# JohannesBuchner/massivedatans

Measured on AMD Instinct MI355X. Metric: likelihood evals/sec across N datasets per constrained draw, higher is better.
Workload: dtype f64

## Files before the change

include/mdns.h:

```cpp
#ifndef MDNS_H
#define MDNS_H

#include <stddef.h>
#include <stdint.h>

#ifdef __cplusplus
extern "C" {
#endif


int mdns_init(int device);
int mdns_device_count(void);
const char *mdns_last_error(void);
int mdns_abi_version(void);


int mdns_gauss_like(const void *x, const void *yy, int ndata, int nx,
                    double A, double mu, double sig, double noise_level,
                    const void *data_mask, void *Lout);

int mdns_muse_like(const void *yy, const void *vv, const void *ypred, const void *data_mask,
                   int ndata, int nx, void *Lout);

int mdns_register_spectra(const void *yy, const void *vv, int ndata, int nx);
// ... 33 lines not shown
int mdns_lines_loglike_batch(mdns_spectra *s, const double *params, int B,
                             const int *row_ids, int M, double *Lout);
int mdns_lines_template_batch(mdns_spectra *s, const double *params, int B, double *out);

int mdns_curve_loglike_batch(mdns_spectra *s, const double *curves, int B, double noise_level,
                             const int *row_ids, int M, double *Lout);

typedef struct mdns_region mdns_region;

mdns_region *mdns_region_create(const double *members, int K, int ndim);
mdns_region *mdns_region_create_bootstrapped(const double *members, int K, int ndim,
                                             const unsigned *packed, int nbootstraps, double *radius);
mdns_region *mdns_region_wrap_dev(const double *d_members, int K, int ndim);
void mdns_region_destroy(mdns_region *r);
double mdns_region_bootstrap_radius(mdns_region *r, const double *chosen, int nbootstraps);
double mdns_region_bootstrap_radius_dev(mdns_region *r, const double *d_chosen, int nbootstraps);
double mdns_region_bootstrap_radius_packed(mdns_region *r, const unsigned *packed, int nbootstraps);
int mdns_region_bootstrap_radius_async(mdns_region *r, const double *d_chosen, int nbootstraps);
int mdns_region_set_radius(mdns_region *r, double maxdistance);
double mdns_region_radius(mdns_region *r);
int mdns_region_count(mdns_region *r, const double *points, int M, int *counts);
int mdns_region_count_dev(mdns_region *r, const double *d_points, int M, int *d_counts);
int mdns_region_count_polled(mdns_region *r, const double *points, int M, int *counts);


typedef struct mdns_joint mdns_joint;

mdns_joint *mdns_joint_create(mdns_spectra *s, int nlive, int shelf_cap);
void mdns_joint_destroy(mdns_joint *j);

int mdns_joint_init_gauss(mdns_joint *j, const double *params, double noise_level);
int mdns_joint_init_muse3(mdns_joint *j, const double *params, const double *jitter);
int mdns_joint_init_curves(mdns_joint *j, const double *curves, double noise_level, const double *jitter);
int mdns_joint_set_live(mdns_joint *j, const double *liveL);
int mdns_joint_get_live(mdns_joint *j, double *liveL);

int mdns_joint_set_running(mdns_joint *j, const int *rows, int nrun);

int mdns_joint_prepare(mdns_joint *j, double *Lmin, int *argmin, unsigned long long *keep);
int mdns_joint_keep_words(const mdns_joint *j);
int mdns_joint_advance(mdns_joint *j);
int mdns_joint_reserve(mdns_joint *j, int shelf_cap);
int mdns_joint_shelf_cap(const mdns_joint *j);

int mdns_joint_draw_gauss(mdns_joint *j, const double *params, int B, double noise_level,
                          const int *row_ids, int M, int *accepted, double *Lrow,
                          unsigned long long *fillbits);
#define MDNS_JOINT_MAX_BATCH 1024
int mdns_joint_score(mdns_joint *j, const double *params, int B, double noise_level,
                     const int *row_ids, int M);
int mdns_joint_commit(mdns_joint *j, int *accepted, double *Lrow, unsigned long long *fillbits);

int mdns_joint_get_thresholds(mdns_joint *j, double *higher, int *shelf_n);


void *mdns_dev_alloc(size_t bytes);
void mdns_dev_free(void *p);
int mdns_h2d(void *dst, const void *src, size_t bytes);
int mdns_d2h(void *dst, const void *src, size_t bytes);
int mdns_d2d(void *dst, const void *src, size_t bytes);
int mdns_sync(void);
int mdns_set_stream(void *hip_stream);

void *mdns_event_create(void);
void mdns_event_destroy(void *ev);
int mdns_event_record(void *ev);
double mdns_event_elapsed_ms(void *ev_start, void *ev_stop);

int mdns_profile(int classes);
int mdns_profile_every(int n);
int mdns_profile_read(int which, long long *launches, double *total_ms);
const char *mdns_profile_kernel(int which);

int mdns_gauss_loglike_batch_dev(mdns_spectra *s, const double *d_params, int B,
                                 double noise_level, const int *d_row_ids, int M,
                                 double *d_Lout);
int mdns_muse_loglike_batch_dev(mdns_spectra *s, const double *d_ypred, int B,
                                const int *d_row_ids, int M, double *d_Lout);
int mdns_muse3_loglike_batch_dev(mdns_spectra *s, const double *d_params, int B,
                                 const int *d_row_ids, int M, double *d_Lout);
int mdns_lines_loglike_batch_dev(mdns_spectra *s, const double *d_params, int B,
                                 const int *d_row_ids, int M, double *d_Lout);

int mdns_curve_loglike_batch_dev(mdns_spectra *s, const double *d_curves, int ldc, int B, double noise_level,
                                 const int *d_row_ids, int M, double *d_Lout);

int mdns_joint_score_dev(mdns_joint *j, const double *d_params, int B, double noise_level,
                         const int *d_row_ids, int M);
int *mdns_joint_flags_dev(mdns_joint *j);
int mdns_joint_commit_dev(mdns_joint *j, const int *d_row_ids, int M);
int mdns_joint_commit_bits_dev(mdns_joint *j, const int *d_row_ids, int M);
const void *mdns_joint_result_dev(mdns_joint *j);
size_t mdns_joint_result_bytes(int M);
int mdns_joint_fetch(mdns_joint *j, int M, int *accepted, unsigned long long *fillbits);
int mdns_joint_prepare_dev(mdns_joint *j);
int mdns_joint_advance_dev(mdns_joint *j);
int mdns_joint_restore_live_dev(mdns_joint *j, const double *d_liveL);
int mdns_joint_undo_advance_dev(mdns_joint *j);
const double *mdns_joint_live_dev(mdns_joint *j);

int mdns_count_within_dev(const double *d_members, int K, int ndim, double maxdistance,
                          const double *d_cands, int M, int *d_counts);
int mdns_bootstrap_round_maxsq_dev(const double *d_members, int K, int ndim,
                                   const double *d_chosen, int nbootstraps,
                                   double *d_round_sq);

// ... 254 lines not shown
```

massivedatans_amd/_lib.py:

```python
import ctypes as C
import os

import numpy as np

PKG_DIR = os.path.dirname(os.path.abspath(__file__))
LIB_PATH = os.path.join(PKG_DIR, "libmdns_hip.so")
DROPIN_DIR = os.path.join(PKG_DIR, "dropin")

ABI_SYMBOLS = (
    "mdns_init", "mdns_device_count", "mdns_last_error", "mdns_abi_version",
    "mdns_gauss_like", "mdns_muse_like", "mdns_register_spectra", "mdns_unregister_spectra",
    "mdns_most_distant_nearest_neighbor", "mdns_is_within_distance_of",
    "mdns_count_within_distance_of", "mdns_bootstrapped_maxdistance",
    "mdns_spectra_create", "mdns_spectra_destroy", "mdns_spectra_ndata", "mdns_spectra_nx",
    "mdns_gauss_loglike_batch", "mdns_muse_loglike_batch", "mdns_muse3_loglike_batch",
    "mdns_region_create", "mdns_region_create_bootstrapped", "mdns_region_wrap_dev", "mdns_region_destroy",
    "mdns_region_bootstrap_radius", "mdns_region_bootstrap_radius_dev", "mdns_region_bootstrap_radius_packed",
    "mdns_region_bootstrap_radius_async", "mdns_region_set_radius",
    "mdns_region_radius", "mdns_region_count", "mdns_region_count_dev", "mdns_region_count_polled",
    "mdns_dev_alloc", "mdns_dev_free", "mdns_h2d", "mdns_d2h", "mdns_d2d", "mdns_sync", "mdns_set_stream",
    "mdns_event_create", "mdns_event_destroy", "mdns_event_record", "mdns_event_elapsed_ms",
    "mdns_profile", "mdns_profile_every", "mdns_profile_read", "mdns_profile_kernel",
    "mdns_gauss_loglike_batch_dev", "mdns_muse_loglike_batch_dev", "mdns_muse3_loglike_batch_dev",
    "mdns_count_within_dev", "mdns_bootstrap_round_maxsq_dev",
    "mdns_joint_create", "mdns_joint_destroy", "mdns_joint_init_gauss", "mdns_joint_init_muse3", "mdns_joint_set_live",
    "mdns_joint_get_live", "mdns_joint_set_running", "mdns_joint_prepare", "mdns_joint_keep_words",
    "mdns_joint_advance", "mdns_joint_reserve", "mdns_joint_shelf_cap", "mdns_joint_draw_gauss", "mdns_joint_score", "mdns_joint_commit",
    "mdns_joint_get_thresholds", "mdns_joint_score_dev", "mdns_joint_flags_dev", "mdns_joint_commit_dev", "mdns_joint_commit_bits_dev",
    "mdns_joint_result_dev", "mdns_joint_result_bytes", "mdns_joint_fetch", "mdns_joint_prepare_dev", "mdns_joint_advance_dev",
    "mdns_joint_restore_live_dev", "mdns_joint_undo_advance_dev", "mdns_joint_live_dev",
    "mdns_groups_create", "mdns_groups_destroy", "mdns_groups_set_ids", "mdns_groups_get_ids",
    "mdns_groups_replace", "mdns_groups_components", "mdns_groups_labels", "mdns_groups_id_labels", "mdns_groups_mean_rounds",
    "mdns_backend_region_create", "mdns_backend_region_destroy", "mdns_backend_region_count",
    "mdns_backend_draw_begin", "mdns_backend_draw_chunk", "mdns_backend_chunk_size",
    "mdns_backend_region_begin", "mdns_backend_region_radius", "mdns_backend_chain_begin", "mdns_backend_chain_end",
    "mdns_backend_draw_score", "mdns_joint_votes_dev", "mdns_backend_draw_commit", "mdns_get_stream",
    "mdns_backend_draw_band", "mdns_backend_draw_band_commit", "mdns_muse_filter_mode", "mdns_muse_filter_stats", "mdns_muse_filter_dev",
    "mdns_backend_draw_band_begin", "mdns_backend_draw_band_ready", "mdns_backend_draw_band_end",
    "mdns_posterior_create", "mdns_posterior_destroy", "mdns_posterior_summary", "mdns_posterior_resample",
    "mdns_posterior_timings",
    "mdns_spectra_set_lines", "mdns_spectra_nparams", "mdns_lines_loglike_batch", "mdns_lines_loglike_batch_dev",
    "mdns_lines_template_batch",
    "mdns_curve_loglike_batch", "mdns_curve_loglike_batch_dev", "mdns_joint_init_curves",
    "mdns_backend_draw_curves", "mdns_backend_draw_curves_dev",
    "mdns_spectra_set_continuum", "mdns_spectra_continuum", "mdns_muse_continuum_fit_batch", "mdns_muse_continuum_fit_batch_dev",
    "mdns_curve_chi2_batch", "mdns_curve_chi2_batch_dev", "mdns_spectra_set_fixed_scale", "mdns_spectra_fixed_scale",
    "mdns_spectra_set_counts", "mdns_spectra_counts", "mdns_curve_poisson_batch", "mdns_curve_poisson_batch_dev",
    "mdns_spectra_set_background", "mdns_spectra_background", "mdns_curve_wstat_batch", "mdns_curve_wstat_batch_dev",
    "mdns_curve_background_batch", "mdns_curve_background_batch_dev",
    "mdns_table_create", "mdns_table_create_los", "mdns_table_destroy", "mdns_table_nparams", "mdns_table_nx", "mdns_table_curves_batch",
    "mdns_table_curves_batch_dev", "mdns_backend_draw_table", "mdns_joint_init_table",
    "mdns_response_create", "mdns_response_destroy", "mdns_response_nx", "mdns_response_nin", "mdns_response_fold_batch",
    "mdns_response_fold_batch_dev", "mdns_spectra_set_response",
    "mdns_sum_create", "mdns_sum_add_table", "mdns_sum_add_powerlaw", "mdns_sum_add_gauss", "mdns_sum_set_attenuation",
    "mdns_sum_destroy", "mdns_sum_nparams", "mdns_sum_nx", "mdns_sum_ncomponents", "mdns_sum_curves_batch",
    "mdns_sum_curves_batch_dev", "mdns_backend_draw_sum", "mdns_joint_init_sum",
)

HOST_ABI_SYMBOLS = (
    "mdns_constrainer_create", "mdns_constrainer_destroy", "mdns_constrainer_forget_region",
    "mdns_constrainer_draw", "mdns_constrainer_stats", "mdns_constrainer_share_stats", "mdns_host_last_error",
    "mdns_host_rng_get_gauss", "mdns_host_rng_set_gauss",
    "mdns_core_create", "mdns_core_destroy", "mdns_core_last_error", "mdns_core_set_host_edges", "mdns_core_set_incremental",
    "mdns_core_set_initial",
    "mdns_core_purge", "mdns_core_fill", "mdns_core_advance", "mdns_core_cut_down", "mdns_core_npoints",
    "mdns_core_nrunning", "mdns_core_pile_u", "mdns_core_pile_x", "mdns_core_get_ids", "mdns_core_get_shelves",
    "mdns_core_get_superpoints", "mdns_core_stats",
)

JOINT_MAX_BATCH = 1024
TABLE_MAX_AXES = 4
TABLE_TILE = 256
TABLE_REDSHIFT = 1
TABLE_AMPLITUDE = 2
TABLE_EXTINCTION = 4
TABLE_BROADEN = 8
TABLE_BROADEN_CUT = 5.0
TABLE_BROADEN_C = float.fromhex("-0x1.bcb7b1526e50ep-3")
SUM_MAX_COMPONENTS = 8


# ... 27 lines not shown
        "mdns_spectra_nx": (i, [vp]),
        "mdns_gauss_loglike_batch": (i, [vp, vp, i, d, vp, i, vp]),
        "mdns_muse_loglike_batch": (i, [vp, vp, i, vp, i, vp]),
        "mdns_muse3_loglike_batch": (i, [vp, vp, i, vp, i, vp]),
        "mdns_region_create": (vp, [vp, i, i]),
        "mdns_region_create_bootstrapped": (vp, [vp, i, i, vp, i, vp]),
        "mdns_region_wrap_dev": (vp, [vp, i, i]),
        "mdns_region_destroy": (None, [vp]),
        "mdns_region_bootstrap_radius": (d, [vp, vp, i]),
        "mdns_region_bootstrap_radius_dev": (d, [vp, vp, i]),
        "mdns_region_bootstrap_radius_packed": (d, [vp, vp, i]),
        "mdns_region_bootstrap_radius_async": (i, [vp, vp, i]),
        "mdns_region_set_radius": (i, [vp, d]),
        "mdns_region_radius": (d, [vp]),
        "mdns_region_count": (i, [vp, vp, i, vp]),
        "mdns_region_count_dev": (i, [vp, vp, i, vp]),
        "mdns_region_count_polled": (i, [vp, vp, i, vp]),
        "mdns_dev_alloc": (vp, [sz]),
        "mdns_dev_free": (None, [vp]),
        "mdns_h2d": (i, [vp, vp, sz]),
        "mdns_d2h": (i, [vp, vp, sz]),
        "mdns_d2d": (i, [vp, vp, sz]),
        "mdns_sync": (i, []),
        "mdns_set_stream": (i, [vp]),
        "mdns_event_create": (vp, []),
        "mdns_event_destroy": (None, [vp]),
        "mdns_event_record": (i, [vp]),
        "mdns_event_elapsed_ms": (d, [vp, vp]),
        "mdns_profile": (i, [i]),
        "mdns_profile_every": (i, [i]),
        "mdns_profile_read": (i, [i, vp, vp]),
        "mdns_profile_kernel": (C.c_char_p, [i]),
        "mdns_gauss_loglike_batch_dev": (i, [vp, vp, i, d, vp, i, vp]),
        "mdns_muse_loglike_batch_dev": (i, [vp, vp, i, vp, i, vp]),
        "mdns_muse3_loglike_batch_dev": (i, [vp, vp, i, vp, i, vp]),
        "mdns_count_within_dev": (i, [vp, i, i, d, vp, i, vp]),
        "mdns_bootstrap_round_maxsq_dev": (i, [vp, i, i, vp, i, vp]),
        "mdns_joint_create": (vp, [vp, i, i]),
        "mdns_joint_destroy": (None, [vp]),
        "mdns_joint_init_gauss": (i, [vp, vp, d]),
        "mdns_joint_init_muse3": (i, [vp, vp, vp]),
        "mdns_joint_set_live": (i, [vp, vp]),
        "mdns_joint_get_live": (i, [vp, vp]),
        "mdns_joint_set_running": (i, [vp, vp, i]),
        "mdns_joint_prepare": (i, [vp, vp, vp, vp]),
        "mdns_joint_keep_words": (i, [vp]),
        "mdns_joint_advance": (i, [vp]),
        "mdns_joint_reserve": (i, [vp, i]),
        "mdns_joint_shelf_cap": (i, [vp]),
        "mdns_joint_draw_gauss": (i, [vp, vp, i, d, vp, i, vp, vp, vp]),
        "mdns_joint_score": (i, [vp, vp, i, d, vp, i]),
        "mdns_joint_commit": (i, [vp, vp, vp, vp]),
        "mdns_joint_get_thresholds": (i, [vp, vp, vp]),
        "mdns_joint_score_dev": (i, [vp, vp, i, d, vp, i]),
        "mdns_joint_flags_dev": (vp, [vp]),
        "mdns_joint_commit_dev": (i, [vp, vp, i]),
        "mdns_joint_commit_bits_dev": (i, [vp, vp, i]),
        "mdns_joint_result_dev": (vp, [vp]),
        "mdns_joint_result_bytes": (sz, [i]),
        "mdns_joint_fetch": (i, [vp, i, vp, vp]),
        "mdns_joint_prepare_dev": (i, [vp]),
        "mdns_joint_advance_dev": (i, [vp]),
        "mdns_joint_restore_live_dev": (i, [vp, vp]),
        "mdns_joint_undo_advance_dev": (i, [vp]),
        "mdns_joint_live_dev": (vp, [vp]),
        "mdns_groups_create": (vp, [i, i]),
        "mdns_groups_destroy": (None, [vp]),
        "mdns_groups_set_ids": (i, [vp, vp]),
        "mdns_groups_get_ids": (i, [vp, vp]),
        "mdns_groups_replace": (i, [vp, vp, vp, vp, i]),
        "mdns_groups_components": (i, [vp, vp, i, C.c_longlong, vp, vp, vp, C.c_longlong, vp]),
        "mdns_groups_labels": (i, [vp, vp, vp]),
        "mdns_groups_id_labels": (i, [vp, vp, vp, C.c_longlong]),
        "mdns_groups_mean_rounds": (d, [vp]),
        "mdns_backend_region_create": (vp, [vp, vp, i, i, vp, i, vp]),
        "mdns_backend_region_destroy": (None, [vp, vp]),
        "mdns_backend_region_count": (i, [vp, vp, vp, i, vp]),
        "mdns_backend_draw_begin": (i, [vp, vp, i]),
        "mdns_backend_draw_chunk": (i, [vp, vp, i, vp, vp, vp, vp]),
        "mdns_backend_chunk_size": (i, [vp, i, i, i]),
        "mdns_backend_region_begin": (vp, [vp, vp, i, i, vp, i]),
        "mdns_backend_region_radius": (i, [vp, vp, vp]),
        "mdns_backend_draw_score": (i, [vp, vp, i, vp]),
        "mdns_joint_votes_dev": (vp, [vp]),
        "mdns_backend_draw_commit": (i, [vp, vp, vp]),
        "mdns_get_stream": (vp, []),
        "mdns_backend_draw_band": (i, [vp, vp, i, vp, vp, vp, vp, vp, vp, vp, i]),
        "mdns_backend_draw_band_commit": (i, [vp, i, vp, vp]),
        "mdns_backend_draw_band_begin": (i, [vp, vp, i, vp]),
        "mdns_backend_draw_band_ready": (i, [vp]),
        "mdns_backend_draw_band_end": (i, [vp, vp, vp, vp, vp, vp, vp, i]),
        "mdns_muse_filter_dev": (i, [vp, vp, i, vp, i, vp, vp, vp]),
        "mdns_muse_filter_mode": (None, [i]),
        "mdns_muse_filter_stats": (None, [vp]),
        "mdns_posterior_create": (vp, [vp, vp, vp, i, i, i]),
        "mdns_posterior_destroy": (None, [vp]),
        "mdns_posterior_summary": (i, [vp, vp, i, vp, vp, vp, vp, vp, vp, vp]),
        "mdns_posterior_resample": (i, [vp, C.c_ulonglong, C.c_longlong, i, vp, vp]),
        "mdns_posterior_timings": (i, [vp, vp]),
        "mdns_spectra_set_lines": (i, [vp, vp, i, i]),
        "mdns_spectra_nparams": (i, [vp]),
        "mdns_lines_loglike_batch": (i, [vp, vp, i, vp, i, vp]),
        "mdns_lines_loglike_batch_dev": (i, [vp, vp, i, vp, i, vp]),
        "mdns_lines_template_batch": (i, [vp, vp, i, vp]),
        "mdns_curve_loglike_batch": (i, [vp, vp, i, d, vp, i, vp]),
        "mdns_curve_loglike_batch_dev": (i, [vp, vp, i, i, d, vp, i, vp]),
# ... 99 lines not shown
```

massivedatans_amd/csrc/mdns_core.hip:

```cpp
#include "mdns_internal.h"
#include <time.h>

#include <atomic>
#include <cmath>
#include <cstdarg>
#include <cstdio>
#include <cstdlib>
#include <cstring>
#include <mutex>
#include <vector>

namespace mdns {

static char g_error[512] = "";

void set_error(const char *fmt, ...)
{
	va_list ap;
	va_start(ap, fmt);
	vsnprintf(g_error, sizeof(g_error), fmt, ap);
	va_end(ap);
	if (getenv("MDNS_VERBOSE")) fprintf(stderr, "[mdns] %s\n", g_error);
}

// ... 215 lines not shown
	return MDNS_HIP(hipStreamSynchronize(c->stream)) ? 0 : 1;
}
extern "C" int mdns_set_stream(void *hip_stream)
{
	Context *c = ctx();
	if (!c) return 1;
	c->stream = hip_stream ? (hipStream_t) hip_stream : c->own_stream;
	return 0;
}
extern "C" void *mdns_get_stream(void)
{
	Context *c = ctx();
	return c ? (void *) c->stream : nullptr;
}
extern "C" void *mdns_event_create(void)
{
	if (!ctx()) return nullptr;
	hipEvent_t ev;
	if (!MDNS_HIP(hipEventCreate(&ev))) return nullptr;
	return (void *) ev;
}
extern "C" void mdns_event_destroy(void *ev) { if (ev) (void) hipEventDestroy((hipEvent_t) ev); }
extern "C" int mdns_event_record(void *ev)
{
	Context *c = ctx();
	if (!c || !ev) return 1;
	return MDNS_HIP(hipEventRecord((hipEvent_t) ev, c->stream)) ? 0 : 1;
}
extern "C" double mdns_event_elapsed_ms(void *a, void *b)
{
	if (!a || !b) return NAN;
	if (!MDNS_HIP(hipEventSynchronize((hipEvent_t) b))) return NAN;
	float ms = 0;
	if (!MDNS_HIP(hipEventElapsedTime(&ms, (hipEvent_t) a, (hipEvent_t) b))) return NAN;
	return (double) ms;
}

extern "C" int mdns_profile(int classes)
{
	if (!ctx()) return 1;
	drain_pending();
	for (int k = 0; k < 4; k++)
		if (classes & (1 << k)) { g_prof_count[k] = 0; g_prof_ms[k] = 0; g_prof_seen[k] = 0; }
	g_profiling = classes & 15;
	return 0;
}
extern "C" int mdns_profile_every(int n)
{
	g_prof_every = n > 1 ? n : 1;
	return 0;
}
static constexpr int kNoteArgs = 4;
struct KernelNote { const char *fmt; int narg; int num[kNoteArgs]; const char *str[kNoteArgs]; };
static KernelNote g_kernel_note[4];
static char g_kernel_name[4][64];
void mdns::note_kernel(int which, const char *fmt, ...)
{
	if (which < 0 || which > 3) return;
	KernelNote &n = g_kernel_note[which];
	n.fmt = fmt;
	n.narg = 0;
	va_list ap;
	va_start(ap, fmt);
	for (const char *p = fmt; *p && n.narg < kNoteArgs; p++) {
		if (*p != '%') continue;
		if (!*++p) break;
		if (*p == 'd') { n.str[n.narg] = nullptr; n.num[n.narg++] = va_arg(ap, int); }
		else if (*p == 's') { n.num[n.narg] = 0; n.str[n.narg++] = va_arg(ap, const char *); }
	}
	va_end(ap);
}
extern "C" const char *mdns_profile_kernel(int which)
{
	if (which < 0 || which > 3) return "";
	const KernelNote &n = g_kernel_note[which];
	char *out = g_kernel_name[which];
	const size_t cap = sizeof g_kernel_name[which];
	size_t len = 0;
	int a = 0;
	out[0] = 0;
	for (const char *p = n.fmt; p && *p && len + 1 < cap; p++) {
		if (*p == '%' && (p[1] == 'd' || p[1] == 's') && a < n.narg) {
			const int w = n.str[a] ? snprintf(out + len, cap - len, "%s", n.str[a]) : snprintf(out + len, cap - len, "%d", n.num[a]);
			len = w < 0 || len + (size_t) w >= cap ? cap - 1 : len + (size_t) w;
			a++;
			p++;
		} else {
			out[len++] = *p;
			out[len] = 0;
		}
	}
	return out;
}
extern "C" int mdns_profile_read(int which, long long *launches, double *total_ms)
{
	if (!ctx() || which < 0 || which > 3) return 1;
	drain_pending();
	if (launches) *launches = g_prof_count[which];
	if (total_ms) *total_ms = g_prof_ms[which];
	return 0;
}

static bool upload_rows(const double *h_src, int ndata, int nx, int layout, double *d_dst, int ld,
                        bool invert)
{
	Context *c = ctx();
	const size_t n = (size_t) ndata * nx;
	DeviceBuffer<double> tmp;
	if (!tmp.make(n)) return false;
	double *const d_tmp = tmp.get();
	bool ok = MDNS_HIP(hipMemcpyAsync(d_tmp, h_src, n * sizeof(double), hipMemcpyHostToDevice, c->stream));
	if (ok) {
		if (layout == MDNS_LAYOUT_CHANNEL_MAJOR) ok = launch_transpose(d_tmp, nx, ndata, d_dst, ld, invert, ndata);
		else ok = launch_copy_rows(d_tmp, nx, ndata, d_dst, ld, invert);
	}
	return MDNS_HIP(hipStreamSynchronize(c->stream)) && ok;
}

extern "C" mdns_spectra *mdns_spectra_create(const double *x, const double *y, const double *v,
                                             int ndata, int nx, int layout)
{
	Context *c = ctx();
	if (!c) return nullptr;
	if (ndata < 0 || nx < 0 || !y || (layout != 0 && layout != 1)) {
		set_error("mdns_spectra_create: bad arguments (ndata=%d nx=%d layout=%d)", ndata, nx, layout);
		return nullptr;
	}
// ... 855 lines not shown
```

massivedatans_amd/csrc/mdns_joint.hip:

```cpp
#include "mdns_internal.h"

#include <cmath>
#include <cstring>
#include <vector>

namespace mdns {

static constexpr int kBlock = 256;
static constexpr int kFlagInts = MDNS_JOINT_MAX_BATCH;
static constexpr int kZeroInts = kFlagInts + (int) (sizeof(JointHeader) / sizeof(int));

static constexpr int kSlices = 16, kHeld = 8;

template <typename T, typename F> __device__ __forceinline__ T over_slices(T v, F f)
{
	v = f(v, __shfl_xor(v, 4));
	v = f(v, __shfl_xor(v, 8));
	v = f(v, __shfl_xor(v, 16));
	v = f(v, __shfl_xor(v, 32));
	return v;
}

__global__ __launch_bounds__(kBlock) void k_joint_prepare(JointArrays st, const int *__restrict__ running, int nrun,
                                                          double *__restrict__ Lmin, int *__restrict__ argmin_run,
// ... 603 lines not shown
	if (j->stat == kCurveNoise) j->noise_level = noise_level;
	if (!sum_curves(j, c, m, params, j->nlive)) return 1;
	return init_from_curves(j, c, jitter);
}

extern "C" int mdns_joint_restore_live_dev(mdns_joint *j, const double *d_liveL)
{
	Context *c = ctx();
	if (!c || !j || !d_liveL) return 1;
	if (!MDNS_HIP(hipMemcpyAsync(j->st.live, d_liveL, (size_t) j->nlive * j->ndata * sizeof(double), hipMemcpyDeviceToDevice, c->stream))) return 1;
	return joint_reset(j);
}

extern "C" int mdns_joint_undo_advance_dev(mdns_joint *j)
{
	Context *c = ctx();
	if (!c || !j) return 1;
	if (!j->prepared) { set_error("mdns_joint_undo_advance_dev: nothing to take back"); return 1; }
	if (j->nrun == 0) return 0;
	joint_new_epoch(j);
	hipLaunchKernelGGL(k_joint_undo_advance, dim3((j->nrun + kBlock - 1) / kBlock), dim3(kBlock), 0, c->stream,
	                   j->st, j->d_running.get(), j->nrun, j->d_argmin.get(), j->d_Lmin.get());
	return MDNS_HIP(hipGetLastError()) ? 0 : 1;
}

extern "C" const double *mdns_joint_live_dev(mdns_joint *j) { return j ? j->st.live : nullptr; }

extern "C" int mdns_joint_set_live(mdns_joint *j, const double *liveL)
{
	Context *c = ctx();
	if (!c || !j || !liveL) return 1;
	if (!MDNS_HIP(hipMemcpyAsync(j->st.live, liveL, (size_t) j->nlive * j->ndata * sizeof(double), hipMemcpyHostToDevice, c->stream))) return 1;
	if (joint_reset(j) != 0) return 1;
	return joint_sync(c) ? 0 : 1;
}

extern "C" int mdns_joint_get_live(mdns_joint *j, double *liveL)
{
	Context *c = ctx();
	if (!c || !j || !liveL) return 1;
	if (!MDNS_HIP(hipMemcpyAsync(liveL, j->st.live, (size_t) j->nlive * j->ndata * sizeof(double), hipMemcpyDeviceToHost, c->stream))) return 1;
	return joint_sync(c) ? 0 : 1;
}

extern "C" int mdns_joint_get_thresholds(mdns_joint *j, double *higher, int *shelf_n)
{
	Context *c = ctx();
	if (!c || !j) return 1;
	if (higher && !MDNS_HIP(hipMemcpyAsync(higher, j->st.higher, (size_t) j->ndata * sizeof(double), hipMemcpyDeviceToHost, c->stream))) return 1;
	if (shelf_n && !MDNS_HIP(hipMemcpyAsync(shelf_n, j->st.shelfn, (size_t) j->ndata * sizeof(int), hipMemcpyDeviceToHost, c->stream))) return 1;
	return joint_sync(c) ? 0 : 1;
}

extern "C" int mdns_joint_set_running(mdns_joint *j, const int *rows, int nrun)
{
	Context *c = ctx();
	if (!c || !j) return 1;
	if (nrun < 0 || nrun > j->ndata || (nrun > 0 && !rows)) { set_error("mdns_joint_set_running: nrun=%d", nrun); return 1; }
	for (int i = 0; i < nrun; i++)
		if (rows[i] < 0 || rows[i] >= j->ndata || (i > 0 && rows[i] <= rows[i - 1])) {
			set_error("mdns_joint_set_running: rows must be ascending indices below %d", j->ndata);
			return 1;
		}
	if (nrun > 0 && (!MDNS_HIP(hipMemcpyAsync(j->d_running.get(), rows, (size_t) nrun * sizeof(int), hipMemcpyHostToDevice, c->stream)) ||
	                 !joint_sync(c))) return 1;
	j->nrun = nrun;
	return 0;
}

extern "C" int mdns_joint_prepare_dev(mdns_joint *j)
{
	Context *c = ctx();
	if (!c || !j) return 1;
	const int kw = keep_words_of(j->cap);
	if (!j->d_keep.fit((size_t) j->ndata * kw)) return 1;
	j->prepared = true;
	if (j->nrun == 0) return 0;
	joint_new_epoch(j);
	hipLaunchKernelGGL(k_joint_prepare, dim3((j->nrun + 15) / 16), dim3(kBlock), 0, c->stream,
	                   j->st, j->d_running.get(), j->nrun, j->d_Lmin.get(), j->d_argmin_run.get(), j->d_argmin.get(), j->d_keep.get(), kw);
	return MDNS_HIP(hipGetLastError()) ? 0 : 1;
}

extern "C" int mdns_joint_prepare(mdns_joint *j, double *Lmin, int *argmin, unsigned long long *keep)
{
	Context *c = ctx();
	if (mdns_joint_prepare_dev(j) != 0) return 1;
	const int kw = keep_words_of(j->cap);
	const size_t n = (size_t) j->nrun;
	if (n == 0) return 0;
	const size_t o1 = n * 8, o2 = o1 + ((n * 4 + 7) & ~(size_t) 7);
	if (!j->h_pin.fit(o2 + n * kw * 8)) return 1;
	char *pin = j->h_pin.get();
	if (!MDNS_HIP(hipMemcpyAsync(pin, j->d_Lmin.get(), n * 8, hipMemcpyDeviceToHost, c->stream)) ||
	    !MDNS_HIP(hipMemcpyAsync(pin + o1, j->d_argmin_run.get(), n * 4, hipMemcpyDeviceToHost, c->stream)) ||
	    !MDNS_HIP(hipMemcpyAsync(pin + o2, j->d_keep.get(), n * kw * 8, hipMemcpyDeviceToHost, c->stream)) ||
	    !joint_sync(c)) return 1;
	if (Lmin) memcpy(Lmin, pin, n * 8);
	if (argmin) memcpy(argmin, pin + o1, n * 4);
	if (keep) memcpy(keep, pin + o2, n * kw * 8);
	int longest = 0;
	const unsigned long long *kwords = (const unsigned long long *) (pin + o2);
	for (size_t r = 0; r < n; r++) {
		int kept = 0;
		for (int w = 0; w < kw; w++) kept += __builtin_popcountll(kwords[r * kw + w]);
		if (kept > longest) longest = kept;
// ... 880 lines not shown
```

massivedatans_amd/csrc/mdns_like.hip:

```cpp
#include "mdns_internal.h"
#include <climits>
#include <cstdlib>

namespace mdns {

static constexpr int kBlock = 256;


__device__ __forceinline__ double swap_add32(double a, double b)
{
	const auto lo = __builtin_amdgcn_permlane32_swap((unsigned) __double2loint(a), (unsigned) __double2loint(b), false, false);
	const auto hi = __builtin_amdgcn_permlane32_swap((unsigned) __double2hiint(a), (unsigned) __double2hiint(b), false, false);
	return __hiloint2double((int) hi[0], (int) lo[0]) + __hiloint2double((int) hi[1], (int) lo[1]);
}
__device__ __forceinline__ double swap_add16(double a, double b)
{
	const auto lo = __builtin_amdgcn_permlane16_swap((unsigned) __double2loint(a), (unsigned) __double2loint(b), false, false);
	const auto hi = __builtin_amdgcn_permlane16_swap((unsigned) __double2hiint(a), (unsigned) __double2hiint(b), false, false);
	return __hiloint2double((int) hi[0], (int) lo[0]) + __hiloint2double((int) hi[1], (int) lo[1]);
}
__device__ __forceinline__ double row_sum(double v)
{
	v += dpp_move<0xb1, 0xf>(v);
	v += dpp_move<0x4e, 0xf>(v);
// ... 257 lines not shown

	for (int k0 = wave * R; k0 < M; k0 += nwaves * R) {
		double2 y[R][NP];
#pragma unroll
		for (int r = 0; r < R; r++) {
			const int k = (k0 + r < M) ? k0 + r : M - 1;
			const int row = rows ? rows[k] : k;
			const double *yr = Y + (size_t) row * ld + ch;
#pragma unroll
			for (int p = 0; p < NP; p++)
				y[r][p] = valid[p] ? *reinterpret_cast<const double2 *>(yr + p * 128) : make_double2(0.0, 0.0);
		}
		for (int b0 = 0; b0 < B; b0 += BT) {
			if (!HOIST) {
#pragma unroll
				for (int b = 0; b < BT; b++) {
					const int bb = (b0 + b < B) ? b0 + b : B - 1;
#pragma unroll
					for (int p = 0; p < NP; p++)
						m[b][p] = *reinterpret_cast<const double2 *>(model + (size_t) bb * ldm + p * 128 + ch);
				}
			}
			double acc[BT][R];
#pragma unroll
			for (int b = 0; b < BT; b++)
#pragma unroll
				for (int r = 0; r < R; r++) {
					double a = 0.0;
#pragma unroll
					for (int p = 0; p < NP; p++) {
						const double d0 = m[b][p].x - y[r][p].x;
						const double d1 = m[b][p].y - y[r][p].y;
						a = fma(d0, d0, a);
						a = fma(d1, d1, a);
					}
					acc[b][r] = a;
				}
			double mine = 0.0;
#pragma unroll
			for (int b = 0; b < BT; b++)
#pragma unroll
				for (int r = 0; r < R; r++) {
					const double s = wave_sum(acc[b][r]);
					if (lane == b * R + r) mine = s;
				}
			if (lane < BT * R) {
				const int b = b0 + lane / R, k = k0 + lane % R;
				if (b < B && k < M) out[(size_t) b * M + k] = mine * scale;
			}
		}
	}
}

__device__ __forceinline__ bool cols_item(int ntiles, int tile_limit, int nq_xcd, int nbt, int cu_slots, int &tile, int &bt)
{
	const int xcd = blockIdx.x & 7;
	const int local = blockIdx.x >> 3;
	const int slot = local % cu_slots, round = local / cu_slots;
	const int nitems = nbt * nq_xcd;
	const int first = (int) ((long long) slot * nitems / cu_slots);
	const int next = (int) ((long long) (slot + 1) * nitems / cu_slots);
	if (first + round >= next) return false;
	bt = (first + round) / nq_xcd;
	const int quad = ((first + round) % nq_xcd) * 8 + xcd;
	const int wpb = blockDim.x >> 6;
	tile = quad * wpb + __builtin_amdgcn_readfirstlane(threadIdx.x >> 6);
	(void) ntiles;
	return tile < tile_limit;
}

template <int BT, int SP, bool RUNTIME_STRIDE, bool DOT = false>
__device__ __forceinline__ void cols_accumulate(const double *__restrict__ YT, int nxp,
                                                const double *mp, int mstride,
                                                const int *__restrict__ rows, int M, int tile, int lane,
                                                int (&k)[SP], double (&acc)[SP][BT])
{
	constexpr int CH = 8;
	const double *yp[SP];
#pragma unroll
	for (int s = 0; s < SP; s++) {
		k[s] = (tile * SP + s) * 64 + lane;
		int col = k[s];
		if (rows) col = rows[k[s] < M ? k[s] : M - 1];
		else if (col >= ((M + 63) & ~63)) col = M - 1;
		yp[s] = YT + ((size_t) (col >> 6) * nxp << 6) + (col & 63);
	}
#pragma unroll
	for (int s = 0; s < SP; s++)
#pragma unroll
		for (int b = 0; b < BT; b++) acc[s][b] = 0.0;
	double ya[SP][CH], yb[SP][CH];
#pragma unroll
	for (int s = 0; s < SP; s++)
#pragma unroll
		for (int c = 0; c < CH; c++) ya[s][c] = yp[s][c * 64];
	const int ms = RUNTIME_STRIDE ? mstride : BT;
	auto stage = [&](const double (&cur)[SP][CH], double (&nxt)[SP][CH], bool last) {
#pragma unroll
		for (int s = 0; s < SP; s++) {
			yp[s] += last ? 0 : CH * 64;
#pragma unroll
			for (int c = 0; c < CH; c++) nxt[s][c] = yp[s][c * 64];
		}
#pragma unroll
		for (int c = 0; c < CH; c++) {
#pragma unroll
			for (int b = 0; b < BT; b++) {
				const double mv = mp[c * ms + b];
#pragma unroll
				for (int s = 0; s < SP; s++) {
					if constexpr (DOT) {
						acc[s][b] = fma(mv, cur[s][c], acc[s][b]);
					} else {
						const double d = mv - cur[s][c];
						acc[s][b] = fma(d, d, acc[s][b]);
					}
				}
			}
		}
		mp += CH * ms;
	};
	int st = nxp / CH;
#pragma unroll 1
	for (; st >= 2; st -= 2) {
		stage(ya, yb, false);
		stage(yb, ya, st == 2);
	}
	if (st == 1) stage(ya, yb, true);
}

template <int BT, int NB>
__device__ __forceinline__ void cols_accumulate_deep(const double *__restrict__ YT, int nxp,
                                                     const double *tpl,
                                                     const int *__restrict__ rows, int M, int tile, int lane,
                                                     int &k, double (&acc)[BT])
{
	constexpr int CH = 8;
	k = tile * 64 + lane;
	int col = k;
	if (rows) col = rows[k < M ? k : M - 1];
	else if (col >= ((M + 63) & ~63)) col = M - 1;
	const double *yp = YT + ((size_t) (col >> 6) * nxp << 6) + (col & 63);
#pragma unroll
	for (int b = 0; b < BT; b++) acc[b] = 0.0;
	const int nst = nxp / CH;
	double y[NB][CH];
#pragma unroll
	for (int i = 0; i < NB - 1; i++) {
		const double *p = yp + (size_t) min(i, nst - 1) * CH * 64;
#pragma unroll
		for (int c = 0; c < CH; c++) y[i][c] = p[c * 64];
	}
#pragma unroll 1
	for (int s0 = 0; s0 < nst; s0 += NB) {
#pragma unroll
		for (int i = 0; i < NB; i++) {
			const int s = s0 + i;
			if (s < nst) {
				const double *p = yp + (size_t) min(s + NB - 1, nst - 1) * CH * 64;
#pragma unroll
				for (int c = 0; c < CH; c++) y[(i + NB - 1) % NB][c] = p[c * 64];
				const double *m = tpl + s * CH * BT;
#pragma unroll
				for (int c = 0; c < CH; c++)
#pragma unroll
					for (int b = 0; b < BT; b++) {
						const double d = m[c * BT + b] - y[i][c];
						acc[b] = fma(d, d, acc[b]);
					}
			}
		}
	}
}

__device__ __forceinline__ void stage_templates(double *__restrict__ dst, const double *__restrict__ src, int n, int stride)
{
	constexpr int U = 4;
	for (int base = 0; base < n; base += U * (int) blockDim.x) {
		double r[U];
#pragma unroll
		for (int u = 0; u < U; u++) {
			const int e = base + u * (int) blockDim.x + (int) threadIdx.x;
			r[u] = src[(size_t) (e < n ? e : n - 1) * stride];
		}
#pragma unroll
		for (int u = 0; u < U; u++) {
			const int e = base + u * (int) blockDim.x + (int) threadIdx.x;
			if (e < n) dst[e] = r[u];
		}
	}
	__syncthreads();
}

template <int BT, int SP>
__global__ __launch_bounds__(kBlock) void k_gauss_cols(
    const double *__restrict__ YT, int nxp, const double *__restrict__ model_t, int B,
    double scale, const int *__restrict__ rows, int M, int ntiles, int nq_xcd, int nbt, int cu_slots, double *__restrict__ out)
{
	const int lane = threadIdx.x & 63;
	int tile, bt;
	if (!cols_item(ntiles, ntiles, nq_xcd, nbt, cu_slots, tile, bt)) return;
	const double *mp = model_t + (size_t) bt * nxp * BT;
	int k[SP];
	double acc[SP][BT];
	cols_accumulate<BT, SP, false>(YT, nxp, mp, BT, rows, M, tile, lane, k, acc);
#pragma unroll
	for (int s = 0; s < SP; s++) {
		if (k[s] < M) {
#pragma unroll
			for (int b = 0; b < BT; b++)
				if (bt * BT + b < B) out[(size_t) (bt * BT + b) * M + k[s]] = acc[s][b] * scale;
		}
	}
}

template <int BT, bool DEEP>
__global__ __launch_bounds__(2 * kBlock) void k_gauss_cols_accept(
    const double *__restrict__ YT, int nxp, const double *__restrict__ model_t, int B,
    double scale, const int *__restrict__ rows, const int *__restrict__ thr_rows, int M,
    int ntiles, int nq_xcd, int nbt, int cu_slots, const double *__restrict__ higher, int *__restrict__ flags,
    JointTrail trail)
{
	const int lane = threadIdx.x & 63;
	int tile, bt;
	int k[1];
	double acc[1][BT];
	if constexpr (DEEP) {
		extern __shared__ __attribute__((aligned(16))) double tpl[];
		const bool mine = cols_item(ntiles, INT_MAX, nq_xcd, nbt, cu_slots, tile, bt);
		if (!mine) return;
		stage_templates(tpl, model_t + (size_t) bt * nxp * BT, nxp * BT, 1);
		if (tile >= ntiles) return;
		cols_accumulate_deep<BT, 4>(YT, nxp, tpl, rows, M, tile, lane, k[0], acc[0]);
	} else {
		if (!cols_item(ntiles, ntiles, nq_xcd, nbt, cu_slots, tile, bt)) return;
		const double *mp = model_t + (size_t) bt * nxp * BT;
		cols_accumulate<BT, 1, false>(YT, nxp, mp, BT, rows, M, tile, lane, k, acc);
	}
	const bool live = k[0] < M;
	const int kk = live ? k[0] : M - 1;
	const double thr = live ? higher[thr_rows ? thr_rows[kk] : kk] : __builtin_nan("");
#pragma unroll
	for (int b = 0; b < BT; b++)
		trail_vote(trail, flags, bt * BT + b, B, ntiles, tile, lane, acc[0][b] * scale, thr);
}

template <int BT>
__global__ __launch_bounds__(2 * kBlock) void k_gauss_cols_filter(
    const double *__restrict__ YT, int nxp, int nx, const double *__restrict__ model_t, const double *__restrict__ msq, int B,
    double scale, const int *__restrict__ rows, const int *__restrict__ thr_rows, int M,
    int ntiles, int nq_xcd, int nbt, int cu_slots, const double *__restrict__ higher, const double *__restrict__ ysq,
    int *__restrict__ flags, JointTrail trail, int *__restrict__ lowest)
{
	const int lane = threadIdx.x & 63;
	int tile, bt;
	int k[1];
	double acc[1][BT];
	if (!cols_item(ntiles, ntiles, nq_xcd, nbt, cu_slots, tile, bt)) return;
	const double *mp = model_t + (size_t) bt * nxp * BT;
	cols_accumulate<BT, 1, false, true>(YT, nxp, mp, BT, rows, M, tile, lane, k, acc);
	const bool live = k[0] < M;
	const int kk = live ? k[0] : M - 1;
	const int d = thr_rows ? thr_rows[kk] : kk;
	const double thr = live ? higher[d] : __builtin_nan("");
	const double yy = ysq[d];
	const double unit = fabs(scale) * (double) (nx + 8) * 0x1p-52;
	unsigned hits = 0, maybes = 0;
#pragma unroll
	for (int b = 0; b < BT; b++) {
		const int cand = bt * BT + b;
		const double mm = msq[cand];
		const double Lf = scale * ((mm - 2.0 * acc[0][b]) + yy);
		const double E4 = 4.0 * unit * ((mm + 2.0 * fabs(acc[0][b])) + yy);
		const bool valid = cand < B;
		if (__ballot(valid && Lf > thr + E4) != 0ull) hits |= 1u << b;
		else if (__ballot(valid && Lf >= thr - E4) != 0ull) maybes |= 1u << b;
	}
	unsigned todo = hits | maybes;
#pragma unroll 1
	while (todo) {
// ... 372 lines not shown
}

bool launch_gauss_model_t(const double *d_x, int nx, const double *d_params, int B, int bt, double *d_model_t,
                          int *d_zero, int nzero)
{
	Context *c = ctx();
	const int nxp = cols_nx(nx);
	const int ntile = (B + bt - 1) / bt;
	const int n = ntile * nxp * bt;
	const int threads = n > nzero ? n : nzero;
	hipLaunchKernelGGL(k_gauss_model_t, dim3((threads + kBlock - 1) / kBlock), dim3(kBlock), 0, c->stream,
	                   d_x, nx, nxp, d_params, B, bt, ntile, d_model_t, d_zero, d_zero ? nzero : 0);
	return launched("k_gauss_model_t");
}

bool launch_gauss_cols(const mdns_spectra *s, const double *d_yT, const double *d_model_t, int bt, int B,
                       double scale, const int *d_rows, int M, double *d_out)
{
	Context *c = ctx();
	constexpr int sp = 1;
	const int ntiles = (M + 64 * sp - 1) / (64 * sp);
	const int nbt = (B + bt - 1) / bt;
	int nq_xcd, cu_slots;
	const int blocks = cols_grid(c, ntiles, nbt, nq_xcd, cu_slots);
	ProfileScope prof(0);
	note_kernel(0, "k_gauss_cols<%d, %d>", bt, (int) sp);
#define COLS_LAUNCH(BT) hipLaunchKernelGGL((k_gauss_cols<BT, sp>), dim3(blocks), dim3(kBlock), 0, c->stream, \
	d_yT, cols_nx(s->nx), d_model_t, B, scale, d_rows, M, ntiles, nq_xcd, nbt, cu_slots, d_out)
	switch (bt) {
	case 16: COLS_LAUNCH(16); break;
	case 8: COLS_LAUNCH(8); break;
	case 4: COLS_LAUNCH(4); break;
	case 2: COLS_LAUNCH(2); break;
	default: COLS_LAUNCH(1); break;
	}
#undef COLS_LAUNCH
	return launched("k_gauss_cols");
}

bool launch_gauss_cols_accept(const mdns_spectra *s, const double *d_yT, const double *d_model_t, int bt, int B,
                              double scale, const int *d_rows, const int *d_thr_rows, int M,
                              const double *d_higher, int *d_flags, const JointTrail &trail)
{
	Context *c = ctx();
	const int ntiles = (M + 63) / 64;
	const int nbt = (B + bt - 1) / bt;
	int nq_xcd, cu_slots;
	const int wpb = 4;
	const int blocks = cols_grid(c, ntiles, nbt, nq_xcd, cu_slots, wpb);
	ProfileScope prof(0);
	note_kernel(0, "k_gauss_cols_accept<%d, %s>", bt, ((long long) ntiles * nbt < 8LL * c->num_cus && bt <= 4 && (size_t) cols_nx(s->nx) * bt * sizeof(double) <= 48 * 1024) ? "true" : "false");
	const size_t tpl_bytes = (size_t) cols_nx(s->nx) * bt * sizeof(double);
	const bool deep = (long long) ntiles * nbt < 8LL * c->num_cus && bt <= 4 && tpl_bytes <= 48 * 1024;
#define ACCEPT_LAUNCH(BT, DEEP) hipLaunchKernelGGL((k_gauss_cols_accept<BT, DEEP>), dim3(blocks), dim3(64 * wpb), DEEP ? tpl_bytes : 0, c->stream, \
	d_yT, cols_nx(s->nx), d_model_t, B, scale, d_rows, d_thr_rows, M, ntiles, nq_xcd, nbt, cu_slots, d_higher, d_flags, trail)
	switch (bt) {
	case 16: ACCEPT_LAUNCH(16, false); break;
	case 8: ACCEPT_LAUNCH(8, false); break;
	case 4: if (deep) ACCEPT_LAUNCH(4, true); else ACCEPT_LAUNCH(4, false); break;
	case 2: if (deep) ACCEPT_LAUNCH(2, true); else ACCEPT_LAUNCH(2, false); break;
	default: if (deep) ACCEPT_LAUNCH(1, true); else ACCEPT_LAUNCH(1, false); break;
	}
#undef ACCEPT_LAUNCH
	return launched("k_gauss_cols_accept");
}

bool launch_row_sumsq(const double *d_y, int ld, int nx, int ndata, double *d_out)
{
	Context *c = ctx();
	if (ndata <= 0) return true;
	hipLaunchKernelGGL(k_row_sumsq, dim3((ndata + kBlock - 1) / kBlock), dim3(kBlock), 0, c->stream, d_y, ld, nx, ndata, d_out);
	return launched("k_row_sumsq");
}

int gauss_filter_pays(const mdns_spectra *s, int M, int B)
{
	static const char *forced = getenv("MDNS_K1_FILTER");
	if (s->d_ysq.get() == nullptr || gauss_cols_tile(M, B) < 8) return 0;
	if (forced && forced[0] == '1') return 1;
	if (forced && forced[0] == '0') return 0;
	const bool listed = cols_nx(s->nx) <= 8 * 32;
	if (forced && forced[0] == 'm') return listed ? 2 : 0;
	return listed && B >= 128 && (long long) M * B >= 8000000LL ? 2 : 0;
}

int gauss_filter_tile(int M, int B)
{
	Context *c = ctx();
	static const char *forced = getenv("MDNS_K1_FILTER_BT");
	if (forced && (atoi(forced) == 8 || atoi(forced) == 16)) return atoi(forced);
	const long long waves = (long long) ((M + 63) / 64) * ((B + 15) / 16);
	return waves >= 2LL * 4 * c->num_cus ? 16 : 8;
}

bool launch_gauss_model_tsq(const double *d_x, int nx, const double *d_params, int B, int bt, double *d_model_t, double *d_msq,
                            int *d_zero, int nzero, double *d_model_g)
{
	Context *c = ctx();
	const int ntile = (B + bt - 1) / bt;
	if (d_model_g && bt != 16) { set_error("launch_gauss_model_tsq: tiled templates come 16 candidates wide"); return false; }
	constexpr int kShares = 4;
	static const char *one = getenv("MDNS_TSQ_SHARES");
	const int ny = one && one[0] == '1' ? 1 : kShares;
	if (ny > 1 && (!c->tsq_part.fit((size_t) ntile * kShares * 64) || !c->tsq_tickets.fit_zeroed((size_t) ntile))) return false;
	hipLaunchKernelGGL(k_gauss_model_tsq, dim3(ntile, ny), dim3(256), 0, c->stream, d_x, nx, cols_nx(nx), d_params, B, bt, d_model_t, d_msq,
	                   d_zero, d_zero ? nzero : 0, d_model_g, tiled16_nx(nx), c->tsq_part.get(), c->tsq_tickets.get());
	return launched("k_gauss_model_tsq");
}

bool launch_tile_rows16(const double *d_y, int ld, int M, int nx, const int *d_rows, double *d_out)
{
	Context *c = ctx();
// ... 206 lines not shown
```

Measured before the change: 31.38 billion.

## Retire rejected draws early in the Gaussian accept kernel via wave ballots

Adds a retiring variant of the column accept kernel. Each wave tests every few stages whether any lane's partial chi-square still exceeds its threshold, and drops draws that can no longer pass; the log-likelihood only decreases as terms accumulate, so the test relies on scale being non-positive. Once half the draws are retired, the wave switches to a sparse loop that broadcasts template values across lanes and only accumulates for draws still alive. Work items are also spread round-robin over CU slots instead of in contiguous ranges. The cost is extra ballot reductions and readlane traffic, some divergence, and more register pressure. A trail-entry counting API and an extra profiling note slot are added.

```diff
diff --git a/include/mdns.h b/include/mdns.h
--- a/include/mdns.h
+++ b/include/mdns.h
@@ -109,6 +109,7 @@
 int mdns_joint_commit(mdns_joint *j, int *accepted, double *Lrow, unsigned long long *fillbits);
 
 int mdns_joint_get_thresholds(mdns_joint *j, double *higher, int *shelf_n);
+int mdns_joint_trail_entries(mdns_joint *j);
 
 
 void *mdns_dev_alloc(size_t bytes);
diff --git a/massivedatans_amd/_lib.py b/massivedatans_amd/_lib.py
--- a/massivedatans_amd/_lib.py
+++ b/massivedatans_amd/_lib.py
@@ -26,7 +26,7 @@
     "mdns_joint_create", "mdns_joint_destroy", "mdns_joint_init_gauss", "mdns_joint_init_muse3", "mdns_joint_set_live",
     "mdns_joint_get_live", "mdns_joint_set_running", "mdns_joint_prepare", "mdns_joint_keep_words",
     "mdns_joint_advance", "mdns_joint_reserve", "mdns_joint_shelf_cap", "mdns_joint_draw_gauss", "mdns_joint_score", "mdns_joint_commit",
-    "mdns_joint_get_thresholds", "mdns_joint_score_dev", "mdns_joint_flags_dev", "mdns_joint_commit_dev", "mdns_joint_commit_bits_dev",
+    "mdns_joint_get_thresholds", "mdns_joint_trail_entries", "mdns_joint_score_dev", "mdns_joint_flags_dev", "mdns_joint_commit_dev", "mdns_joint_commit_bits_dev",
     "mdns_joint_result_dev", "mdns_joint_result_bytes", "mdns_joint_fetch", "mdns_joint_prepare_dev", "mdns_joint_advance_dev",
     "mdns_joint_restore_live_dev", "mdns_joint_undo_advance_dev", "mdns_joint_live_dev",
     "mdns_groups_create", "mdns_groups_destroy", "mdns_groups_set_ids", "mdns_groups_get_ids",
@@ -160,6 +160,7 @@
         "mdns_joint_score": (i, [vp, vp, i, d, vp, i]),
         "mdns_joint_commit": (i, [vp, vp, vp, vp]),
         "mdns_joint_get_thresholds": (i, [vp, vp, vp]),
+        "mdns_joint_trail_entries": (i, [vp]),
         "mdns_joint_score_dev": (i, [vp, vp, i, d, vp, i]),
         "mdns_joint_flags_dev": (vp, [vp]),
         "mdns_joint_commit_dev": (i, [vp, vp, i]),
diff --git a/massivedatans_amd/csrc/mdns_core.hip b/massivedatans_amd/csrc/mdns_core.hip
--- a/massivedatans_amd/csrc/mdns_core.hip
+++ b/massivedatans_amd/csrc/mdns_core.hip
@@ -291,11 +291,11 @@
 }
 static constexpr int kNoteArgs = 4;
 struct KernelNote { const char *fmt; int narg; int num[kNoteArgs]; const char *str[kNoteArgs]; };
-static KernelNote g_kernel_note[4];
-static char g_kernel_name[4][64];
+static KernelNote g_kernel_note[5];
+static char g_kernel_name[5][64];
 void mdns::note_kernel(int which, const char *fmt, ...)
 {
-	if (which < 0 || which > 3) return;
+	if (which < 0 || which > 4) return;
 	KernelNote &n = g_kernel_note[which];
 	n.fmt = fmt;
 	n.narg = 0;
@@ -311,7 +311,7 @@
 }
 extern "C" const char *mdns_profile_kernel(int which)
 {
-	if (which < 0 || which > 3) return "";
+	if (which < 0 || which > 4) return "";
 	const KernelNote &n = g_kernel_note[which];
 	char *out = g_kernel_name[which];
 	const size_t cap = sizeof g_kernel_name[which];
diff --git a/massivedatans_amd/csrc/mdns_joint.hip b/massivedatans_amd/csrc/mdns_joint.hip
--- a/massivedatans_amd/csrc/mdns_joint.hip
+++ b/massivedatans_amd/csrc/mdns_joint.hip
@@ -679,6 +679,20 @@
 	return joint_sync(c) ? 0 : 1;
 }
 
+extern "C" int mdns_joint_trail_entries(mdns_joint *j)
+{
+	Context *c = ctx();
+	if (!c || !j) return -1;
+	if (!j->trail_valid || j->last_B <= 0 || j->scored_M <= 0) return 0;
+	const size_t n = (size_t) j->last_B * ((j->scored_M + 63) / 64);
+	if (n > j->d_trail_stamp.cap()) return -1;
+	std::vector<int> stamps(n);
+	if (!MDNS_HIP(hipMemcpyAsync(stamps.data(), j->d_trail_stamp.get(), n * sizeof(int), hipMemcpyDeviceToHost, c->stream)) || !joint_sync(c)) return -1;
+	int count = 0;
+	for (size_t i = 0; i < n; i++) count += stamps[i] == j->trail_stamp;
+	return count;
+}
+
 extern "C" int mdns_joint_set_running(mdns_joint *j, const int *rows, int nrun)
 {
 	Context *c = ctx();
diff --git a/massivedatans_amd/csrc/mdns_like.hip b/massivedatans_amd/csrc/mdns_like.hip
--- a/massivedatans_amd/csrc/mdns_like.hip
+++ b/massivedatans_amd/csrc/mdns_like.hip
@@ -333,17 +333,25 @@
 	}
 }
 
-__device__ __forceinline__ bool cols_item(int ntiles, int tile_limit, int nq_xcd, int nbt, int cu_slots, int &tile, int &bt)
+__device__ __forceinline__ bool cols_item(int ntiles, int tile_limit, int nq_xcd, int nbt, int cu_slots, int &tile, int &bt,
+                                          bool spread = false)
 {
 	const int xcd = blockIdx.x & 7;
 	const int local = blockIdx.x >> 3;
 	const int slot = local % cu_slots, round = local / cu_slots;
 	const int nitems = nbt * nq_xcd;
-	const int first = (int) ((long long) slot * nitems / cu_slots);
-	const int next = (int) ((long long) (slot + 1) * nitems / cu_slots);
-	if (first + round >= next) return false;
-	bt = (first + round) / nq_xcd;
-	const int quad = ((first + round) % nq_xcd) * 8 + xcd;
+	int item;
+	if (spread) {
+		item = round * cu_slots + slot;
+		if (item >= nitems) return false;
+	} else {
+		const int first = (int) ((long long) slot * nitems / cu_slots);
+		const int next = (int) ((long long) (slot + 1) * nitems / cu_slots);
+		if (first + round >= next) return false;
+		item = first + round;
+	}
+	bt = item / nq_xcd;
+	const int quad = (item % nq_xcd) * 8 + xcd;
 	const int wpb = blockDim.x >> 6;
 	tile = quad * wpb + __builtin_amdgcn_readfirstlane(threadIdx.x >> 6);
 	(void) ntiles;
@@ -410,6 +418,106 @@
 	if (st == 1) stage(ya, yb, true);
 }
 
+__device__ __forceinline__ double lane_value(double v, int l)
+{
+	return __hiloint2double(__builtin_amdgcn_readlane(__double2hiint(v), l), __builtin_amdgcn_readlane(__double2loint(v), l));
+}
+template <int BT>
+__device__ __forceinline__ unsigned cols_accumulate_retire(const double *__restrict__ YT, int nxp, const double *mp,
+                                                           const int *__restrict__ rows, int M, int tile, int lane,
+                                                           double scale, double thr, unsigned alive, double (&acc)[BT])
+{
+	constexpr int CH = 8;
+	int col = tile * 64 + lane;
+	if (rows) col = rows[col < M ? col : M - 1];
+	else if (col >= ((M + 63) & ~63)) col = M - 1;
+	const double *yp = YT + ((size_t) (col >> 6) * nxp << 6) + (col & 63);
+#pragma unroll
+	for (int b = 0; b < BT; b++) acc[b] = 0.0;
+	double ya[CH], yb[CH];
+#pragma unroll
+	for (int c = 0; c < CH; c++) ya[c] = yp[c * 64];
+	auto prefetch = [&](double (&nxt)[CH], bool last) {
+		yp += last ? 0 : CH * 64;
+#pragma unroll
+		for (int c = 0; c < CH; c++) nxt[c] = yp[c * 64];
+	};
+	auto test = [&]() {
+#pragma unroll
+		for (int b = 0; b < BT; b++)
+			if ((alive >> b & 1u) && __ballot(acc[b] * scale > thr) == 0ull) alive &= ~(1u << b);
+	};
+	const int nst = nxp / CH;
+	int s = 0;
+	{
+		const double *m = mp;
+		auto stage_all = [&](const double (&cur)[CH], double (&nxt)[CH], bool last) {
+			prefetch(nxt, last);
+#pragma unroll
+			for (int c = 0; c < CH; c++)
+#pragma unroll
+				for (int b = 0; b < BT; b++) {
+					const double d = m[c * BT + b] - cur[c];
+					acc[b] = fma(d, d, acc[b]);
+				}
+			m += CH * BT;
+		};
+		auto test_all = [&]() {
+#pragma unroll
+			for (int b = 0; b < BT; b++)
+				if (__ballot(acc[b] * scale > thr) == 0ull) alive &= ~(1u << b);
+		};
+#pragma unroll 1
+		for (; s + 2 <= nst && 2 * __builtin_popcount(alive) > BT; s += 2) {
+			stage_all(ya, yb, false);
+			stage_all(yb, ya, s + 2 == nst);
+			test_all();
+		}
+		if (s + 1 == nst && 2 * __builtin_popcount(alive) > BT) {
+			stage_all(ya, yb, true);
+			return alive;
+		}
+		if (alive == 0u) return 0u;
+	}
+	constexpr int NB = 2, NE = CH * BT, NR = (NE + 63) / 64;
+	const double *tp = mp + (NE < 64 ? lane & (NE - 1) : lane);
+	double t[NB][NR];
+	auto templates = [&](double (&dst)[NR], int stage) {
+		const double *p = tp + (size_t) min(stage, nst - 1) * NE;
+#pragma unroll
+		for (int r = 0; r < NR; r++) dst[r] = p[r * 64];
+	};
+	auto stage_live = [&](const double (&cur)[CH], double (&nxt)[CH], const double (&tv)[NR], bool last) {
+		prefetch(nxt, last);
+#pragma unroll
+		for (int b = 0; b < BT; b++) {
+			if (alive >> b & 1u) {
+#pragma unroll
+				for (int c = 0; c < CH; c++) {
+					const double d = lane_value(tv[(c * BT + b) / 64], (c * BT + b) % 64) - cur[c];
+					acc[b] = fma(d, d, acc[b]);
+				}
+			}
+		}
+	};
+#pragma unroll
+	for (int i = 0; i < NB - 1; i++) templates(t[i], s + i);
+#pragma unroll 1
+	for (; s < nst; s += NB) {
+#pragma unroll
+		for (int i = 0; i < NB; i++) {
+			if (s + i < nst) {
+				templates(t[(i + NB - 1) % NB], s + i + NB - 1);
+				if (i & 1) stage_live(yb, ya, t[i], s + i == nst - 1);
+				else stage_live(ya, yb, t[i], s + i == nst - 1);
+				test();
+				if (alive == 0u) return 0u;
+			}
+		}
+	}
+	return alive;
+}
+
 template <int BT, int NB>
 __device__ __forceinline__ void cols_accumulate_deep(const double *__restrict__ YT, int nxp,
                                                      const double *tpl,
@@ -495,7 +603,7 @@
 	}
 }
 
-template <int BT, bool DEEP>
+template <int BT, bool DEEP, bool RETIRE = false>
 __global__ __launch_bounds__(2 * kBlock) void k_gauss_cols_accept(
     const double *__restrict__ YT, int nxp, const double *__restrict__ model_t, int B,
     double scale, const int *__restrict__ rows, const int *__restrict__ thr_rows, int M,
@@ -506,7 +614,21 @@
 	int tile, bt;
 	int k[1];
 	double acc[1][BT];
-	if constexpr (DEEP) {
+	if constexpr (RETIRE) {
+		static_assert(!DEEP, "the retiring form is a form of the big launches");
+		if (!cols_item(ntiles, ntiles, nq_xcd, nbt, cu_slots, tile, bt, true)) return;
+		k[0] = tile * 64 + lane;
+		const bool live = k[0] < M;
+		const int kk = live ? k[0] : M - 1;
+		const double thr = live ? higher[thr_rows ? thr_rows[kk] : kk] : __builtin_nan("");
+		const int left = B - bt * BT;
+		unsigned alive = left >= BT ? (1u << BT) - 1u : (1u << left) - 1u;
+		alive = cols_accumulate_retire<BT>(YT, nxp, model_t + (size_t) bt * nxp * BT, rows, M, tile, lane, scale, thr, alive, acc[0]);
+#pragma unroll
+		for (int b = 0; b < BT; b++)
+			if (alive >> b & 1u) trail_vote(trail, flags, bt * BT + b, B, ntiles, tile, lane, acc[0][b] * scale, thr);
+		return;
+	} else if constexpr (DEEP) {
 		extern __shared__ __attribute__((aligned(16))) double tpl[];
 		const bool mine = cols_item(ntiles, INT_MAX, nq_xcd, nbt, cu_slots, tile, bt);
 		if (!mine) return;
@@ -985,12 +1107,15 @@
 	note_kernel(0, "k_gauss_cols_accept<%d, %s>", bt, ((long long) ntiles * nbt < 8LL * c->num_cus && bt <= 4 && (size_t) cols_nx(s->nx) * bt * sizeof(double) <= 48 * 1024) ? "true" : "false");
 	const size_t tpl_bytes = (size_t) cols_nx(s->nx) * bt * sizeof(double);
 	const bool deep = (long long) ntiles * nbt < 8LL * c->num_cus && bt <= 4 && tpl_bytes <= 48 * 1024;
-#define ACCEPT_LAUNCH(BT, DEEP) hipLaunchKernelGGL((k_gauss_cols_accept<BT, DEEP>), dim3(blocks), dim3(64 * wpb), DEEP ? tpl_bytes : 0, c->stream, \
+	static const char *no_retire = getenv("MDNS_K1_RETIRE");
+	const bool retire = !(no_retire && no_retire[0] == '0') && scale <= 0.0;
+	note_kernel(4, "k_gauss_cols_accept<%d, %s, %s>", bt, deep ? "true" : "false", retire && !deep && bt >= 4 ? "true" : "false");
+#define ACCEPT_LAUNCH(BT, DEEP, ...) hipLaunchKernelGGL((k_gauss_cols_accept<BT, DEEP, ##__VA_ARGS__>), dim3(blocks), dim3(64 * wpb), DEEP ? tpl_bytes : 0, c->stream, \
 	d_yT, cols_nx(s->nx), d_model_t, B, scale, d_rows, d_thr_rows, M, ntiles, nq_xcd, nbt, cu_slots, d_higher, d_flags, trail)
 	switch (bt) {
-	case 16: ACCEPT_LAUNCH(16, false); break;
-	case 8: ACCEPT_LAUNCH(8, false); break;
-	case 4: if (deep) ACCEPT_LAUNCH(4, true); else ACCEPT_LAUNCH(4, false); break;
+	case 16: if (retire) ACCEPT_LAUNCH(16, false, true); else ACCEPT_LAUNCH(16, false); break;
+	case 8: if (retire) ACCEPT_LAUNCH(8, false, true); else ACCEPT_LAUNCH(8, false); break;
+	case 4: if (deep) ACCEPT_LAUNCH(4, true); else if (retire) ACCEPT_LAUNCH(4, false, true); else ACCEPT_LAUNCH(4, false); break;
 	case 2: if (deep) ACCEPT_LAUNCH(2, true); else ACCEPT_LAUNCH(2, false); break;
 	default: if (deep) ACCEPT_LAUNCH(1, true); else ACCEPT_LAUNCH(1, false); break;
 	}
```

Result: faster. 37.19 billion, median of 6 (+18.5%).
